# entn-at/tf-kaldi-speaker

Measured on AMD Instinct MI355X. Metric: utterances/sec x-vector extraction (30-dim x 300-frame), higher is better.
Workload: dtype f16+fp6-cross(f32-split); 1 GPU; tdnn x-vector (tdnn6_dense), statistics_pooling, 256 utt/GPU/step of 300 frames x 30 dims; batch_per_gpu=256, frames=300, node=tdnn6_dense, precision=f16f6, parallelism=utterance-shard x1, launch=stream launches

## Files before the change

### tf-kaldi-speaker_amd/csrc/pool.hip

```cpp
#include "xv_epilogue.h"

namespace xv {


__device__ __forceinline__ float act_apply(float v, int act, float alpha) {
  switch (act) {
    case ACT_RELU: return fmaxf(v, 0.0f);
    case ACT_LRELU: return fmaxf(v, kLreluAlpha * v);
    case ACT_PRELU: return fmaxf(v, 0.0f) + alpha * (v - fabsf(v)) * 0.5f;
    case ACT_TANH: return tanhf(v);
    default: return v;
  }
}

__device__ __forceinline__ float wave_sum(float v) {
#pragma unroll
  for (int o = 32; o > 0; o >>= 1) v += __shfl_xor(v, o, 64);
  return v;
}
__device__ __forceinline__ float wave_max(float v) {
#pragma unroll
  for (int o = 32; o > 0; o >>= 1) v = fmaxf(v, __shfl_xor(v, o, 64));
  return v;
}
// ... 40 lines not shown
  return hipGetLastError();
}

__global__ __launch_bounds__(256) void pool_finalize_kernel(const float* __restrict__ part, int C,
                                                            const int32_t* __restrict__ off0, int ctx,
                                                            const int32_t* __restrict__ slotbase,
                                                            float* __restrict__ out, int64_t ldo) {
  const int b = blockIdx.y;
  const int n = blockIdx.x * 256 + threadIdx.x;
  if (n >= C) return;
  const int r0 = off0[b] - b * ctx, r1 = off0[b + 1] - (b + 1) * ctx;
  const int t0 = r0 >> 6, t1 = (r1 - 1) >> 6;
  const int64_t base = (int64_t)slotbase[b];
  float s = 0.f;
  for (int t = t0; t <= t1; ++t) s += part[((base + t) * 2) * C + n];
  const float mean = s / (float)(r1 - r0);
  float m2 = 0.f;
  for (int t = t0; t <= t1; ++t) {
    const int ni = min(r1, (t + 1) << 6) - max(r0, t << 6);
    const float d = part[((base + t) * 2) * C + n] / (float)ni - mean;
    m2 += part[((base + t) * 2 + 1) * C + n] + (float)ni * d * d;
  }
  float var = m2 / (float)(r1 - r0);
  var = var <= kVarFloor ? kVarFloor : var;
  out[(int64_t)b * ldo + n] = mean;
  out[(int64_t)b * ldo + C + n] = sqrtf(var);
}

hipError_t launch_pool_finalize(const float* part, int C, const int32_t* off0, int B, int ctx,
                                const int32_t* slotbase, float* out, int64_t ldo, hipStream_t s) {
  if (B <= 0) return hipSuccess;
  hipLaunchKernelGGL(pool_finalize_kernel, dim3((C + 255) / 256, B), dim3(256), 0, s, part, C, off0, ctx, slotbase,
                     out, ldo);
  return hipGetLastError();
}

template <bool VEC>
__global__ __launch_bounds__(256) void stat_pool_kernel(const float* __restrict__ x, int64_t ldx, int C,
                                                        const int32_t* __restrict__ off0, int ctx,
                                                        float* __restrict__ out, int64_t ldo) {
  __shared__ float red[4][64];
  const int b = blockIdx.y;
  const int tid = threadIdx.x, lane = tid & 63, wave = tid >> 6;
  const int cl = tid & 15, rs = tid >> 4;
  const int col = blockIdx.x * 64 + cl * 4;
  const int r0 = off0[b] - b * ctx, r1 = off0[b + 1] - (b + 1) * ctx;
  const int L = r1 - r0;
  const float invL = 1.0f / (float)L;

  auto load4 = [&](int r) -> f32x4 {
    const float* p = x + (int64_t)r * ldx + col;
    if (VEC) {
      if (col < C) return *reinterpret_cast<const f32x4*>(p);
      return f32x4{0.f, 0.f, 0.f, 0.f};
    }
    f32x4 v;
#pragma unroll
    for (int e = 0; e < 4; ++e) v[e] = (col + e < C) ? p[e] : 0.f;
    return v;
  };
  auto block_sum = [&](f32x4 v) -> f32x4 {
#pragma unroll
    for (int e = 0; e < 4; ++e) {
      v[e] += __shfl_xor(v[e], 16, 64);
      v[e] += __shfl_xor(v[e], 32, 64);
    }
// ... 410 lines not shown
```

### tf-kaldi-speaker_amd/csrc/xv_kernels.h

```cpp
#pragma once
#include <hip/hip_runtime.h>
#include <stdint.h>

#include <string>

#include "../../include/xvec_hip.h"

namespace xv {

enum Act : int { ACT_NONE = 0, ACT_RELU = 1, ACT_LRELU = 2, ACT_PRELU = 3, ACT_TANH = 4 };

constexpr float kLreluAlpha = 0.2f;
constexpr int kFlagWords = 8, kUttSmallWord = 4, kFeatMaxSlots = 32768;
constexpr float kVarFloor = 1e-12f;

struct GemmArgs {
  const float* X;
  int64_t ldx;
  int cin;
  int M;
  int K;
  int N;
  const float* Wt;
  int Kpad;
// ... 40 lines not shown
  int64_t att_ld = 0;
  int att_heads = 0;
  const float* pool_w = nullptr;
  int pool_heads = 0;
  int pool_split = 0;
  int pool_dvh = 0;
  int pool_odim = 0;
};

hipError_t launch_gemm_f32(const GemmArgs& a, bool aligned, hipStream_t s);

int gemm_f32_ksplit(int M, int Kpad, int Npad);

int64_t gemm_bf16x3_tail_plan(int M, int Kpad, int Npad, int w, int* tail_mt, int* splits, int cb_quant = 1);

hipError_t launch_im2col_sb(const float* x, int64_t ldx, int cin, int w, int64_t rows, void* out_sb, int ldsb, int f16,
                            int* ovf, hipStream_t s);

hipError_t launch_gemm_bf16x3(const GemmArgs& a, hipStream_t s);
hipError_t launch_gemm_f16f6(const GemmArgs& a, hipStream_t s);
hipError_t launch_f6v2_tail_reduce(const GemmArgs& a, int nMain, hipStream_t s);
hipError_t launch_f6_from_sb(const void* sb, void* out, int64_t rows, int nblk, hipStream_t s);

hipError_t launch_build_rowmap(const int32_t* off0, int B, int ctx_in, int w, int32_t* rowmap, int M,
                               hipStream_t s);

hipError_t launch_stat_pool(const float* x, int64_t ldx, int C, const int32_t* off0, int B, int ctx,
                            float* out, int64_t ldo, hipStream_t s);

hipError_t launch_build_row2utt(const int32_t* off0, int B, int ctx, int32_t* row2utt, int M, hipStream_t s);
hipError_t launch_pool_finalize(const float* part, int C, const int32_t* off0, int B, int ctx,
                                const int32_t* slotbase, float* out, int64_t ldo, hipStream_t s);

hipError_t launch_build_rowmap_grid(const int32_t* off0, int B, int rows_per_t, int Fout, int So, int cover, int32_t* rowmap,
                                    int64_t M, hipStream_t s);
hipError_t launch_build_rowmap_grid_ts(const int32_t* off_in, const int32_t* off_out, int B, int rows_per_t, int Fout, int So,
                                       int ktime, int32_t* rowmap, int64_t M, hipStream_t s);
hipError_t launch_build_rowmap_grid_compact(const int32_t* off_in, const int32_t* off_out, int B, int Sin, int So, int Fout,
                                            int sw, int st, int ktime, int32_t* arow, int32_t* rowmap, int64_t M, int64_t Mpad,
                                            hipStream_t s);
hipError_t launch_grid_zero_border(const int32_t* off0, int B, int64_t frames, int F, int S, int chunks_y, int chunks_sb,
                                   float* y, void* ysb, hipStream_t s);
hipError_t launch_build_rowmap_rows(const int32_t* off0, int B, int32_t* rowmap, int64_t M, hipStream_t s);
hipError_t launch_build_rowmap_trows(const int32_t* off0, int B, int So, int32_t* rowmap, int64_t M, hipStream_t s);
hipError_t launch_build_rowmap_interior(const int32_t* off0, int B, int F, int S, int32_t* rowmap, int64_t M, hipStream_t s);
hipError_t launch_im2col2d_sb(const float* x, int64_t ldx, const int32_t* off0, int B, int F, int S, int64_t P, void* out_sb,
                              int f16, int* ovf, hipStream_t s);
hipError_t launch_im2col2d_f32(const float* x, int64_t ldx, const int32_t* off0, int B, int F, int S, int64_t P, float* out,
                               hipStream_t s);
hipError_t launch_conv0_direct(const float* x, int64_t ldx, const int32_t* off0, int B, int F, int S, int C, int64_t P,
                               const float* wdir, int act, const float* alpha, float* y, void* ysb, int ldsb, int f16, int* ovf,
                               float sb_mul, hipStream_t s);
hipError_t launch_grid_maxpool3x3(const float* x, const int32_t* off0, int B, int F, int S, int C, int64_t P, float* y,
                                  void* ysb, int ldsb, int f16, int* ovf, float sb_mul, hipStream_t s);
hipError_t launch_grid_unpad_n(const float* grid, const int32_t* off0, int B, int F, int S, int C, int64_t frames, float* out,
                               hipStream_t s);

hipError_t launch_cmn_select(const float* x, int64_t ld, int dim, const int32_t* off, int B, double* prefix,
                             const int32_t* src, int64_t out_rows, int window, int center, int min_window, float* out,
                             hipStream_t s);

int mfcc_create(const xv_mfcc_opts* opts, int device, xv_mfcc** out, std::string* err);
void mfcc_destroy(xv_mfcc* m);
int mfcc_num_frames(const xv_mfcc* m, int64_t num_samples, int64_t* out);
int mfcc_device(const xv_mfcc* m);
int mfcc_num_ceps(const xv_mfcc* m);
// ... 81 lines not shown
```

### tf-kaldi-speaker_amd/csrc/xvec_api.hip

```cpp
#include <hip/hip_runtime.h>

#include <algorithm>
#include <cmath>
#include <cstdarg>
#include <cstdio>
#include <cstring>
#include <map>
#include <mutex>
#include <string>
#include <vector>

#include "../../include/xvec_hip.h"
#include "xv_kernels.h"

using namespace xv;

namespace {

constexpr double kBnEps = 1e-3;
constexpr int kSlackRows = 512;
constexpr int kAlign = 256;

thread_local std::string g_last_error;

// ... 88 lines not shown

struct Op {
  int kind = OP_GEMM;
  int layer = -1;
  int in0 = -1, in1 = -1;
  int out = -1;
  int bnvec = -1;
};

struct Node {
  std::string name;
  int op = -1;
  int stage = -1;
  bool att_weights = false;
};

}

struct xv_handle {
  xv_model_desc desc{};
  int device = 0;
  bool finalized = false;
  std::string err;
  std::mutex mu;
  std::mutex err_mu;
  std::mutex prof_mu;
  int opt_pool_fusion = 1;
  int opt_tail_split = 1;
  int opt_onetap_f6_notail = 1;
  int opt_grid_f6 = 1;
  int opt_slab3 = 1;
  int opt_grid_compact = 1;
  int opt_att_fusion = 1;
  int opt_profile_dominant = 0;
  std::mutex pool_mu;
  std::vector<DevBuf> pool;
  size_t pool_bytes = 0;
  std::map<std::string, HostTensor> tensors;
  std::vector<Layer> layers;
  std::vector<Value> values;
  std::vector<Op> ops;
  std::vector<Node> nodes;
  DevBuf query;
  DevBuf ovf_flag;
  DevBuf query_eff;
  int key_npad = 0;
  int att_dk_h = 0, att_dk = 0, att_dv = 0;
  int final_ctx = 14;
  std::string post_bn_scope, post_alpha_name;
  DevBuf post_vec;
  int pool_dim = 0;
  struct ProfRec { hipEvent_t e0, e1; const xv_plan* plan; int step; };
  bool profiling = false;
  std::vector<hipEvent_t> prof_pool;
  size_t prof_next = 0;
  std::vector<ProfRec> prof_recs;
  int prof_forwards = 0;
};

struct PlanStep {
  int op = -1;
  int stage = -1;
  bool to_out = false;
  int64_t out_off = -1;
  int64_t out_sb_off = -1;
  int64_t in0_off = -1, in1_off = -1;
  int64_t in0_sb_off = -1;
  int64_t rows_in = 0, rows_out = 0;
  int M = 0;
  int rowmap = -1;
  int64_t scratch_off = -1;
  int64_t scratch2_off = -1;
  int ksplit = 1;
  int tail_mt = 0;
  bool fuse_pool = false;
  int lvl_in = 0, lvl_out = 0;
  int64_t frames_out = 0;
  bool grid_cover = false;
  bool out_f6 = false;
  bool trows = false;
  bool in_f6 = false;
  bool compact = false;
  int arow = -1;
  int fuse_att = 0;
  int64_t att_w_off = -1;
  int64_t att_s0_off = -1;
  int64_t att_ld = 0;
  bool unpad_to_out = false;
  int64_t flops = 0, bytes = 0;
};

struct xv_plan {
  xv_handle* h = nullptr;
  xv_plan_info info{};
  std::vector<int32_t> offsets;
  std::vector<int32_t> offsets_slotbase;
  DevBuf d_offsets;
  std::vector<int32_t> lvl_offsets[4];
  DevBuf d_lvl[4];
  const int32_t* dev_offsets(int level) const {
    return static_cast<const int32_t*>(level > 0 ? d_lvl[level].p : d_offsets.p);
  }
  DevBuf d_rowmaps;
  std::vector<int64_t> rowmap_off;
  std::vector<PlanStep> steps;
  DevBuf d_row2utt;
  DevBuf d_slotbase;
  int64_t pool_slots = 0;
  bool uniform_len = true;
  int uniform_L = 0;
  int dominant_step = 0;
};

namespace {

int fail(xv_handle* h, int code, const char* fmt, ...) {
  char buf[512];
  va_list ap;
  va_start(ap, fmt);
  vsnprintf(buf, sizeof(buf), fmt, ap);
  va_end(ap);
  if (h) {
    std::lock_guard<std::mutex> lk(h->err_mu);
    h->err = buf;
  }
  g_last_error = buf;
  return code;
}

#define XV_HIP(h, expr)                                                                              \
  do {                                                                                               \
    hipError_t _e = (expr);                                                                          \
    if (_e != hipSuccess)                                                                            \
      return fail((h), XV_ERR_HIP, "%s failed: %s (%s:%d)", #expr, hipGetErrorString(_e), __FILE__,  \
                  __LINE__);                                                                         \
  } while (0)

int64_t align_up(int64_t v, int64_t a) { return (v + a - 1) / a * a; }

constexpr size_t kPoolMaxBuffers = 96, kPoolMaxBytes = (size_t)1 << 30;
// ... 735 lines not shown
    }
    if (h->desc.att_apply_nonlinear) {
      const int n = h->pool_dim;
      std::vector<double> s, t;
      bn_fold(h, h->post_bn_scope, n, s, t);
      std::vector<float> vec((size_t)3 * n, 0.f);
      for (int i = 0; i < n; ++i) { vec[i] = (float)s[i]; vec[(size_t)n + i] = (float)t[i]; }
      if (!h->post_alpha_name.empty()) {
        const auto& a = T(h, h->post_alpha_name).data;
        for (int i = 0; i < n; ++i) vec[(size_t)2 * n + i] = a[i];
      }
      XV_HIP(h, h->post_vec.alloc(vec.size() * sizeof(float)));
      XV_HIP(h, hipMemcpy(h->post_vec.p, vec.data(), vec.size() * sizeof(float), hipMemcpyHostToDevice));
    }
  }
  XV_HIP(h, h->ovf_flag.alloc((kFlagWords + kFeatMaxSlots) * sizeof(int)));
  XV_HIP(h, hipMemset(h->ovf_flag.p, 0, (kFlagWords + kFeatMaxSlots) * sizeof(int)));
  XV_HIP(h, hipDeviceSynchronize());
  for (auto& kv : h->tensors) { kv.second.data.clear(); kv.second.data.shrink_to_fit(); }
  h->finalized = true;
  return XV_OK;
}

int xv_set_option(xv_handle* h, const char* name, int value) {
  if (!h || !name) return fail(h, XV_ERR_INVALID, "xv_set_option: null argument");
  std::lock_guard<std::mutex> lk(h->mu);
  if (!strcmp(name, "pool_fusion")) h->opt_pool_fusion = value != 0;
  else if (!strcmp(name, "tail_split")) h->opt_tail_split = value != 0;
  else if (!strcmp(name, "att_fusion")) h->opt_att_fusion = value != 0;
  else if (!strcmp(name, "slab3")) h->opt_slab3 = value != 0;
  else if (!strcmp(name, "onetap_f6_notail")) h->opt_onetap_f6_notail = value != 0;
  else if (!strcmp(name, "grid_f6")) h->opt_grid_f6 = value != 0;
  else if (!strcmp(name, "grid_compact")) h->opt_grid_compact = value != 0;
  else if (!strcmp(name, "profile_dominant")) h->opt_profile_dominant = value != 0;
  else return fail(h, XV_ERR_INVALID, "xv_set_option: unknown option '%s'", name);
  return XV_OK;
}

int xv_check_overflow(xv_handle* h, int reset) {
  if (!h) return fail(nullptr, XV_ERR_INVALID, "xv_check_overflow: null handle");
  if (!h->finalized || !h->ovf_flag.p) return 0;
  DeviceGuard g(h->device);
  std::vector<int32_t> w((size_t)kFlagWords + kFeatMaxSlots);
  XV_HIP(h, hipMemcpy(w.data(), h->ovf_flag.p, w.size() * sizeof(int32_t), hipMemcpyDeviceToHost));
  int32_t v[2] = {w[0], w[1]};
  for (int i = 0; i < kFeatMaxSlots; ++i) v[1] = std::max(v[1], w[(size_t)kFlagWords + i]);
  if (w[kUttSmallWord]) v[1] = w[kUttSmallWord];
  if (reset) XV_HIP(h, hipMemset(h->ovf_flag.p, 0, w.size() * sizeof(int32_t)));
  return xv_flags_decode(v);
}

int xv_flags_decode(const int32_t* flags) {
  if (!flags) return XV_ERR_INVALID;
  if (flags[0]) return 1;
  if (flags[1] > 0) {
    float mx;
    memcpy(&mx, &flags[1], 4);
    if (mx < 0.00390625f) return 2;
  }
  return 0;
}

int xv_flags_async(xv_handle* h, int32_t* host_flags, void* stream) {
  if (!h || !host_flags) return fail(h, XV_ERR_INVALID, "xv_flags_async: null argument");
  if (!h->finalized || !h->ovf_flag.p) { host_flags[0] = host_flags[1] = 0; return XV_OK; }
  DeviceGuard g(h->device);
// ... 150 lines not shown
  auto arena_free = [&](int64_t off, int64_t size) {
    free_list.push_back({off, size});
    std::sort(free_list.begin(), free_list.end(), [](const Block& a, const Block& b) { return a.off < b.off; });
    for (size_t i = 0; i + 1 < free_list.size();)
      if (free_list[i].off + free_list[i].size == free_list[i + 1].off) {
        free_list[i].size += free_list[i + 1].size;
        free_list.erase(free_list.begin() + i + 1);
      } else {
        ++i;
      }
  };

  std::vector<char> want_f32(h->values.size(), 0), want_sb(h->values.size(), 0);
  for (int o : order) {
    const Op& op = h->ops[o];
    const bool split_in = op.kind == OP_GEMM && h->layers[op.layer].use_split;
    if (op.in0 > 0) (split_in ? want_sb : want_f32)[op.in0] = 1;
    if (op.in1 > 0) want_f32[op.in1] = 1;
  }
  std::vector<int64_t> voff_sb(h->values.size(), -1), vsize_sb(h->values.size(), 0);

  int fused_value = -1;
  for (int o : order) {
    const Op& op = h->ops[o];
    if (op.kind != OP_STAT_POOL || op.in0 <= 0 || producer[op.in0] < 0) continue;
    const Op& prod = h->ops[producer[op.in0]];
    if (prod.kind != OP_GEMM || producer[op.in0] == node.op) continue;
    const Layer& L = h->layers[prod.layer];
    int readers = 0;
    for (int o2 : order)
      if (h->ops[o2].in0 == op.in0 || h->ops[o2].in1 == op.in0) ++readers;
    if (readers == 1 && L.w == 1 && (L.cout & 3) == 0 && h->opt_pool_fusion) fused_value = op.in0;
  }
  const int slot_value = fused_value >= 0 ? fused_value : att_pool_value;
  if (slot_value >= 0) {
    const int ctx = h->values[slot_value].ctx;
    const std::vector<int32_t>& so = lvl[h->values[slot_value].tlevel];
    std::vector<int32_t> slotbase(batch);
    int64_t nslots = 0;
    for (int b = 0; b < batch; ++b) {
      const int r0 = so[b] - b * ctx, r1 = so[b + 1] - (b + 1) * ctx;
      const int t0 = r0 >> 6, t1 = (r1 - 1) >> 6;
      slotbase[b] = (int32_t)(nslots - t0);
      nslots += t1 - t0 + 1;
    }
    p->pool_slots = nslots;
    p->offsets_slotbase = std::move(slotbase);
  }

  int64_t total_flops = 0;
  int64_t rowmap_elems = 0;
  for (size_t s = 0; s < order.size(); ++s) {
    const Op& op = h->ops[order[s]];
    PlanStep st;
    int64_t step_scratch = 0, step_scratch2 = 0;
    st.op = order[s];
    st.to_out = (order[s] == node.op);
    st.rows_in = op.in0 >= 0 ? value_rows(h, op.in0, Fl, batch) : 0;
    st.rows_out = value_rows(h, op.out, Fl, batch);
    st.lvl_in = op.in0 >= 0 ? h->values[op.in0].tlevel : 0;
    st.lvl_out = h->values[op.out].tlevel;
    st.frames_out = Fl[st.lvl_out];
    st.in0_off = op.in0 == 0 ? -2 : (op.in0 > 0 ? voff[op.in0] : -1);
    st.in0_sb_off = op.in0 > 0 ? voff_sb[op.in0] : -1;
    st.in1_off = op.in1 > 0 ? voff[op.in1] : -1;
    if (op.kind == OP_GEMM) {
      const Layer& L = h->layers[op.layer];
      st.stage = st.to_out ? node.stage : L.final_stage();
      const int64_t padded_rows = Fl[st.lvl_in] + 2 * (int64_t)batch;
      if (L.mode == 0) st.M = (int)(st.rows_in - (L.w - 1));
      else if (L.mode == 1 && L.use_f6) {
        st.trows = true;
        st.M = (int)padded_rows;
      }
      else if ((L.mode == 1 || L.mode == 2) && L.use_split && h->opt_grid_compact &&
               st.rows_in * (int64_t)sb_ld(L.cin) * 4 < ((int64_t)1 << 32)) {
        st.compact = true;
        st.M = (int)(Fl[st.lvl_out] * L.Fout);
      }
      else if (L.mode == 1 || L.mode == 2) st.M = (int)(padded_rows * (h->values[op.in0].grid_S / L.sw));
      else if (L.mode == 3) st.M = (int)padded_rows;
      else st.M = (int)(padded_rows * h->values[op.out].grid_S);
      if (st.compact || st.trows) st.grid_cover = false;
      else if (L.mode == 1 || L.mode == 2) st.grid_cover = L.st == 1 && h->values[op.in0].grid_S / L.sw == h->values[op.out].grid_S;
      else if (L.mode == 4) st.grid_cover = true;
      if (L.w > 1 || L.mode != 0) {
        st.rowmap = (int)p->rowmap_off.size();
        p->rowmap_off.push_back(rowmap_elems);
        rowmap_elems += align_up(st.M, 64);
        if (st.compact) {
          st.arow = (int)p->rowmap_off.size();
          p->rowmap_off.push_back(rowmap_elems);
          rowmap_elems += align_up(st.M, 128);
        }
      }
      const int64_t valid_out = L.mode == 0 ? st.rows_out : Fl[st.lvl_out] * (L.mode == 3 ? 1 : L.Fout);
      st.flops = 2 * valid_out * (int64_t)L.cout * L.K();
      st.bytes = 4 * (st.rows_in * L.cin + st.rows_out * L.cout + (int64_t)L.K() * L.cout);
      int64_t scratch = 0;
      if (L.mode == 4) {
        scratch = ((int64_t)st.M + kSlackRows) * 32 * 4;
      } else if (L.im2col) {
        scratch = L.cin_pad ? (st.rows_in + kSlackRows) * (int64_t)L.cin_pad * 4 : (st.M + kSlackRows) * (int64_t)L.Kpad * 4;
      } else if (!L.use_split && op.out != fused_value) {
        st.ksplit = gemm_f32_ksplit(st.M, L.Kpad, L.Npad);
        if (st.ksplit > 1) scratch = (int64_t)st.ksplit * st.M * L.Npad * 4;
      } else if (L.use_f6) {
        scratch = (st.rows_in + kSlackRows) * (int64_t)sb_ld(L.cin) * 4;
        if (h->opt_tail_split && op.in1 <= 0 && L.mode == 0) {
          const int64_t part = gemm_bf16x3_tail_plan(st.M, L.Kpad, L.Npad, L.w, &st.tail_mt, &st.ksplit, 4);
          if (part > 0) {
            step_scratch2 = align_up(part, kAlign);
            st.scratch2_off = arena_alloc(step_scratch2);
          }
        }
      } else if (L.use_split && L.mode == 0 && op.out != fused_value && op.in1 <= 0 && h->opt_tail_split &&
                 order[s] != key_prod && order[s] != val_prod) {
        scratch = gemm_bf16x3_tail_plan(st.M, L.Kpad, L.Npad, L.w, &st.tail_mt, &st.ksplit);
      }
      if (scratch > 0) {
        step_scratch = align_up(scratch, kAlign);
        st.scratch_off = arena_alloc(step_scratch);
      }
    } else if (op.kind == OP_AFFINE_ACT) {
      st.stage = st.to_out ? node.stage : 2;
      st.bytes = 8 * st.rows_out * h->values[op.out].cols;
    } else if (op.kind == OP_ATT_POOL && val_prod >= 0) {
      st.fuse_att = 1;
      st.bytes = 4 * (p->pool_slots * (2 * (h->pool_dim / 2) + h->desc.att_num_heads) + st.rows_out * h->values[op.out].cols);
      st.flops = 8 * p->pool_slots * (h->pool_dim / 2);
    } else if (op.kind == OP_STAT_POOL || op.kind == OP_ATT_POOL) {
      st.bytes = 4 * (st.rows_in * h->values[op.in0].cols + st.rows_out * h->values[op.out].cols);
      st.flops = 4 * st.rows_in * h->values[op.in0].cols;
      if (op.kind == OP_STAT_POOL && op.in0 == fused_value) {
        st.fuse_pool = true;
        st.bytes = 4 * (p->pool_slots * 2 * h->values[op.in0].cols + st.rows_out * h->values[op.out].cols);
// ... 40 lines not shown
        st.fuse_att = 2;
        vsize[op.out] = align_up(p->pool_slots * 2 * (int64_t)(h->pool_dim / 2) * 4, kAlign);
        voff[op.out] = arena_alloc(vsize[op.out]);
        st.out_off = voff[op.out];
        st.bytes = 4 * (st.rows_in * h->layers[op.layer].cin + (int64_t)h->layers[op.layer].K() * h->layers[op.layer].cout +
                        st.rows_out * h->desc.att_num_heads) + vsize[op.out];
        for (const PlanStep& prev : p->steps)
          if (h->ops[prev.op].kind == OP_ATT_SOFTMAX) { st.att_w_off = prev.out_off; st.att_s0_off = prev.att_s0_off; }
      } else if (op.out == fused_value) {
        st.fuse_pool = true;
        vsize[op.out] = align_up(p->pool_slots * 2 * (int64_t)h->values[op.out].cols * 4, kAlign);
        voff[op.out] = arena_alloc(vsize[op.out]);
        st.out_off = voff[op.out];
      } else if (want_f32[op.out] || node.att_weights) {
        vsize[op.out] = value_bytes(h, op.out, Fl, batch);
        if (op.kind == OP_ATT_SCORES && val_prod >= 0)
          vsize[op.out] = align_up(st.rows_out * (int64_t)h->desc.att_num_heads * 4, kAlign) +
                          align_up(p->pool_slots * (int64_t)h->desc.att_num_heads * 4, kAlign) + kAlign;
        voff[op.out] = arena_alloc(vsize[op.out]);
        st.out_off = voff[op.out];
      }
      if (want_sb[op.out]) {
        vsize_sb[op.out] = value_sb_bytes(h, op.out, Fl, batch);
        voff_sb[op.out] = arena_alloc(vsize_sb[op.out]);
        st.out_sb_off = voff_sb[op.out];
      }
    }
    if (op.kind == OP_ATT_POOL && val_prod >= 0)
      for (const PlanStep& prev : p->steps)
        if (h->ops[prev.op].kind == OP_ATT_SOFTMAX) st.att_s0_off = prev.att_s0_off;
    p->steps.push_back(st);
    if (step_scratch > 0) arena_free(st.scratch_off, step_scratch);
    if (step_scratch2 > 0) arena_free(st.scratch2_off, step_scratch2);
    for (int in : {op.in0, op.in1})
      if (in > 0 && last_use[in] == (int)s) {
        if (vsize[in] > 0) { arena_free(voff[in], vsize[in]); vsize[in] = 0; }
        if (vsize_sb[in] > 0) { arena_free(voff_sb[in], vsize_sb[in]); vsize_sb[in] = 0; }
      }
  }

  for (size_t i = 0; i < p->steps.size(); ++i)
    if (p->steps[i].flops > p->steps[p->dominant_step].flops) p->dominant_step = (int)i;

  for (PlanStep& cs : p->steps) {
    const Op& cop = h->ops[cs.op];
    if (cop.kind != OP_GEMM || !h->layers[cop.layer].use_f6) continue;
    const bool grid = h->layers[cop.layer].mode == 1;
    if (cs.in_f6) continue;
    int readers = 0;
    bool all_f6 = true;
    PlanStep* prod = nullptr;
    for (PlanStep& os : p->steps) {
      const Op& o = h->ops[os.op];
      if (o.in0 == cop.in0 || (!grid && o.in1 == cop.in0)) {
        ++readers;
        if (o.kind != OP_GEMM || !h->layers[o.layer].use_f6 || o.in0 != cop.in0) all_f6 = false;
      }
      if (o.out == cop.in0) prod = &os;
    }
    if (!prod || !all_f6 || (grid && readers != 1)) continue;
    const Op& pop = h->ops[prod->op];
    if (pop.kind != OP_GEMM) continue;
    const Layer& PL = h->layers[pop.layer];
    if (prod->to_out || prod->out_sb_off < 0 || prod->stage != PL.final_stage()) continue;
    if (grid) {
      const bool gather = PL.mode == 1 && !PL.use_f6 && PL.use_split && prod->compact && prod->out_off < 0 && pop.in1 <= 0;
// ... 62 lines not shown
      const Layer& L = h->layers[op.layer];
      const int ctx_in = h->values[op.in0].ctx;
      const int32_t* doff = p->dev_offsets(st.lvl_in);
      int32_t* rm = static_cast<int32_t*>(p->d_rowmaps.p) + p->rowmap_off[st.rowmap];
      if (L.mode == 0) e = launch_build_rowmap(doff, batch, ctx_in, L.w, rm, st.M, s);
      else if (st.trows) e = launch_build_rowmap_trows(doff, batch, h->values[op.out].grid_S, rm, st.M, s);
      else if (st.compact)
        e = launch_build_rowmap_grid_compact(doff, p->dev_offsets(st.lvl_out), batch, h->values[op.in0].grid_S,
                                             h->values[op.out].grid_S, L.Fout, L.sw, L.st, L.mode == 1 ? 3 : 1,
                                             static_cast<int32_t*>(p->d_rowmaps.p) + p->rowmap_off[st.arow], rm, st.M,
                                             align_up(st.M, 128), s);
      else if ((L.mode == 1 || L.mode == 2) && L.st == 2)
        e = launch_build_rowmap_grid_ts(doff, p->dev_offsets(st.lvl_out), batch, h->values[op.in0].grid_S / L.sw, L.Fout,
                                        h->values[op.out].grid_S, L.mode == 1 ? 3 : 1, rm, st.M, s);
      else if (L.mode == 1 || L.mode == 2)
        e = launch_build_rowmap_grid(doff, batch, h->values[op.in0].grid_S / L.sw, L.Fout, h->values[op.out].grid_S,
                                     st.grid_cover ? 1 : 0, rm, st.M, s);
      else if (L.mode == 3) e = launch_build_rowmap_rows(doff, batch, rm, st.M, s);
      else e = launch_build_rowmap_interior(doff, batch, L.Fout, h->values[op.out].grid_S, rm, st.M, s);
      if (e != hipSuccess) return bail(e, "build_rowmap");
    }
  }
  if (slot_value >= 0) {
    const int ctx = h->values[slot_value].ctx;
    const int64_t rows = value_rows(h, slot_value, Fl, batch);
    if ((e = pool_take(h, (size_t)rows * 4, p->d_row2utt)) != hipSuccess) return bail(e, "hipMalloc(row2utt)");
    if ((e = pool_take(h, (size_t)batch * 4, p->d_slotbase)) != hipSuccess) return bail(e, "hipMalloc(slotbase)");
    if ((e = hipMemcpyAsync(p->d_slotbase.p, p->offsets_slotbase.data(), (size_t)batch * 4, hipMemcpyHostToDevice, s)) != hipSuccess)
      return bail(e, "hipMemcpyAsync(slotbase)");
    if ((e = launch_build_row2utt(p->dev_offsets(h->values[slot_value].tlevel), batch, ctx,
                                  static_cast<int32_t*>(p->d_row2utt.p), (int)rows, s)) != hipSuccess)
      return bail(e, "build_row2utt");
  }
  *out = p;
  return XV_OK;
}

int xv_plan_query(const xv_plan* p, xv_plan_info* info) {
  if (!p || !info) return XV_ERR_INVALID;
  *info = p->info;
  return XV_OK;
}

void xv_plan_destroy(xv_plan* p) {
  if (!p) return;
  {
    DeviceGuard g(p->h->device);
    pool_give(p->h, p->d_offsets);
    for (int k = 1; k < 4; ++k) pool_give(p->h, p->d_lvl[k]);
    pool_give(p->h, p->d_rowmaps);
    pool_give(p->h, p->d_row2utt);
    pool_give(p->h, p->d_slotbase);
  }
  delete p;
}

static const char* step_name(const xv_handle* h, const PlanStep& st) {
  const Op& op = h->ops[st.op];
  switch (op.kind) {
    case OP_GEMM: {
      const Layer& L = h->layers[op.layer];
      if (!L.ep[ST_AFFINE].empty()) return L.ep[ST_AFFINE].c_str();
      const size_t a = L.kernel_name.find('/'), b = L.kernel_name.rfind('/');
      static thread_local std::string tmp;
      tmp = (a != std::string::npos && b > a) ? L.kernel_name.substr(a + 1, b - a - 1) : L.kernel_name;
      return tmp.c_str();
    }
    case OP_STAT_POOL: return "stat_pool";
    case OP_ATT_SCORES: return "att_scores";
    case OP_ATT_SOFTMAX: return "att_softmax";
    case OP_ATT_POOL: return "att_pool";
    case OP_AFFINE_ACT: return "att_post";
    case OP_L2_SCALE: return "l2_scale";
    case OP_GRID_MAXPOOL: return "conv0_max";
    default: return "op";
  }
}

static int run_plan(xv_handle* h, const xv_plan* p, const float* feats, int feat_ld, float* out, int64_t out_cap,
                    void* workspace, int64_t ws_bytes, hipStream_t s) {
  if (!h || !p) return fail(h, XV_ERR_INVALID, "xv_forward: null handle/plan");
  if (p->h != h) return fail(h, XV_ERR_INVALID, "xv_forward: plan belongs to another handle");
  if (!feats || !out) return fail(h, XV_ERR_INVALID, "xv_forward: null feature/output pointer");
  if (feat_ld < h->desc.feat_dim) return fail(h, XV_ERR_INVALID, "xv_forward: feat_ld %d < feature_dim %d", feat_ld, h->desc.feat_dim);
  if (out_cap < p->info.out_rows * p->info.out_cols)
// ... 84 lines not shown
          a.ntaps = L.mode == 1 ? 3 : 1;
          a.ktap = L.mode == 1 ? 3 * L.cin : (L.mode == 2 ? L.cin : L.Fin * L.cin);
          a.tap_stride = Sin * L.cin;
          a.cin = a.K;
        }
        if (op.in1 > 0) { a.R = in_ptr(st.in1_off); a.ldr = L.cout; }
        if (st.fuse_att == 1) {
          a.Y = nullptr;
          a.att_part = reinterpret_cast<float*>(ws + st.out_off);
          a.att_ld = st.att_ld;
          a.att_heads = d.att_num_heads;
          a.att_q = static_cast<const float*>(h->query_eff.p);
        } else if (st.fuse_att == 2) {
          a.Y = nullptr;
          a.pool_part = reinterpret_cast<float*>(ws + st.out_off);
          a.pool_row2utt = static_cast<const int32_t*>(p->d_row2utt.p);
          a.pool_slotbase = static_cast<const int32_t*>(p->d_slotbase.p);
          a.pool_w = reinterpret_cast<const float*>(ws + st.att_w_off);
          a.pool_heads = d.att_num_heads;
          a.pool_split = d.att_split_value;
          a.pool_dvh = d.att_split_value ? L.cout / d.att_num_heads : L.cout;
          a.pool_odim = h->pool_dim / 2;
        }
        if (st.fuse_pool) {
          a.Y = nullptr;
          a.pool_part = reinterpret_cast<float*>(ws + st.out_off);
          a.pool_row2utt = static_cast<const int32_t*>(p->d_row2utt.p);
          a.pool_slotbase = static_cast<const int32_t*>(p->d_slotbase.p);
        }
        if (st.out_sb_off >= 0) {
          a.Ysb = ws + st.out_sb_off;
          a.ldsb = sb_ld(L.cout);
          if (st.out_off < 0 && !st.to_out) a.Y = nullptr;
        }
        if (L.mode == 4) {
          if (st.scratch_off < 0) return fail(h, XV_ERR_STATE, "conv0 has no scratch");
          a.cin = 32; a.K = 32;
          const bool direct = L.use_split && !st.to_out && st.stage == L.final_stage() && L.cout % 8 == 0 &&
                              (st.out_sb_off < 0 || L.cout % 32 == 0) && L.cout <= 256 && L.wdir.p;
          if (direct) {
            XV_HIP(h, launch_conv0_direct(feats, feat_ld, off, B, L.Fout, vo.grid_S, L.cout, st.M, static_cast<const float*>(L.wdir.p),
                                          L.act, L.d_alpha(), st.out_off >= 0 ? reinterpret_cast<float*>(ws + st.out_off) : nullptr,
                                          st.out_sb_off >= 0 ? ws + st.out_sb_off : nullptr, sb_ld(L.cout), f16,
                                          static_cast<int*>(h->ovf_flag.p), a.sb_mul, s));
            break;
          }
          if (L.use_split) {
            XV_HIP(h, launch_im2col2d_sb(feats, feat_ld, off, B, L.Fout, vo.grid_S, st.M, ws + st.scratch_off, f16, static_cast<int*>(h->ovf_flag.p), s));
            a.Xsb = ws + st.scratch_off; a.ldsbx = 32; a.Wsb = L.wsb.p; a.Wfr = L.wfr.p;
            XV_HIP(h, launch_gemm_bf16x3(a, s));
          } else {
            XV_HIP(h, launch_im2col2d_f32(feats, feat_ld, off, B, L.Fout, vo.grid_S, st.M, reinterpret_cast<float*>(ws + st.scratch_off), s));
            a.X = reinterpret_cast<const float*>(ws + st.scratch_off); a.ldx = 32;
            XV_HIP(h, launch_gemm_f32(a, true, s));
          }
          if (st.unpad_to_out)
            XV_HIP(h, launch_grid_unpad_n(reinterpret_cast<const float*>(ws + st.out_off), off_out, B, vo.grid_F, vo.grid_S, vo.cols,
                                          st.frames_out, out, s));
          break;
        }
        if (L.im2col) {
          if (st.scratch_off < 0) return fail(h, XV_ERR_STATE, "im2col layer has no scratch");
          if (L.cin_pad) {
            XV_HIP(h, launch_im2col_sb(feats, feat_ld, L.cin, 1, st.rows_in, ws + st.scratch_off, L.cin_pad, f16,
                                       static_cast<int*>(h->ovf_flag.p), s));
            if (f16) XV_HIP(h, launch_feat_utt_guard(feats, feat_ld, L.cin, off, B, static_cast<int*>(h->ovf_flag.p), s));
// ... 600 lines not shown
```

Baseline: 216,300 utterances/s.

## Fuse pooling finalize into following dense GEMM with split-K last-block reduction

Adds a head_fused kernel that computes per-utterance mean/std from pooled partial sums directly into LDS and immediately multiplies them by the next dense layer's weights using fp32 MFMA. The channel dimension is split across blocks, and a per-utterance-tile atomic counter lets the last block sum the slab partials and apply the affine epilogue and activation. This removes the separate pool_finalize launch, the write and re-read of the pooled stats, and the standalone GEMM launch. In exchange it adds scratch slabs, atomic counters that must be reset, and cross-block synchronisation.

Result: slower. 214,000 utterances/s (-1.0%).

```diff
diff --git a/tf-kaldi-speaker_amd/csrc/pool.hip b/tf-kaldi-speaker_amd/csrc/pool.hip
--- a/tf-kaldi-speaker_amd/csrc/pool.hip
+++ b/tf-kaldi-speaker_amd/csrc/pool.hip
@@ -96,6 +96,201 @@
   if (B <= 0) return hipSuccess;
   hipLaunchKernelGGL(pool_finalize_kernel, dim3((C + 255) / 256, B), dim3(256), 0, s, part, C, off0, ctx, slotbase,
                      out, ldo);
+  return hipGetLastError();
+}
+
+constexpr int kHeadU = 16, kHeadMaxCS = 256, kHeadBatch = 8;
+
+void head_fused_shape(int B, int C, int* nU, int* nS, int* CS) {
+  const int nu = (B + kHeadU - 1) / kHeadU;
+  int target = 256 / nu;
+  target = target < 1 ? 1 : (target > 32 ? 32 : target);
+  int cs = ((C + target - 1) / target + 15) / 16 * 16;
+  cs = cs < 16 ? 16 : (cs > kHeadMaxCS ? kHeadMaxCS : cs);
+  *nU = nu;
+  *CS = cs;
+  *nS = (C + cs - 1) / cs;
+}
+
+int64_t head_fused_scratch_bytes(int B, int C, int Npad) {
+  int nU, nS, CS;
+  head_fused_shape(B, C, &nU, &nS, &CS);
+  return (int64_t)nU * nS * kHeadU * Npad * 4;
+}
+
+int head_fused_counters(int B) { return (B + kHeadU - 1) / kHeadU; }
+
+struct HeadPair {
+  const float* col;
+  int r0, r1;
+  int64_t base;
+};
+
+__device__ __forceinline__ void head_finish(const HeadPair& q, int C, const float (&sv)[kHeadBatch], const float (&mv)[kHeadBatch],
+                                            float& mean_out, float& std_out) {
+  const int r0 = q.r0, r1 = q.r1;
+  const int t0 = r0 >> 6, t1 = (r1 - 1) >> 6, n = t1 - t0 + 1;
+  const float L = (float)(r1 - r0);
+  auto term = [&](int t, float s1, float m2, float mean) {
+    const int ni = min(r1, (t + 1) << 6) - max(r0, t << 6);
+    const float d = s1 / (float)ni - mean;
+    return m2 + (float)ni * d * d;
+  };
+  float s = 0.f, m2 = 0.f;
+#pragma unroll
+  for (int i = 0; i < kHeadBatch; ++i) s += i < n ? sv[i] : 0.f;
+  for (int t = t0 + kHeadBatch; t <= t1; ++t) s += q.col[((q.base + t) * 2) * C];
+  const float mean = s / L;
+#pragma unroll
+  for (int i = 0; i < kHeadBatch; ++i) m2 += i < n ? term(t0 + i, sv[i], mv[i], mean) : 0.f;
+  for (int t = t0 + kHeadBatch; t <= t1; ++t) m2 += term(t, q.col[((q.base + t) * 2) * C], q.col[((q.base + t) * 2 + 1) * C], mean);
+  float var = m2 / L;
+  var = var <= kVarFloor ? kVarFloor : var;
+  mean_out = mean;
+  std_out = sqrtf(var);
+}
+
+__global__ __launch_bounds__(256) void head_fused_kernel(GemmArgs p, const float* __restrict__ part, int C,
+                                                         const int32_t* __restrict__ off0, int ctx,
+                                                         const int32_t* __restrict__ slotbase, int* __restrict__ counters,
+                                                         int nU, int nS, int CS) {
+  __shared__ __attribute__((aligned(16))) float As[kHeadU * (2 * kHeadMaxCS + 4) + 4];
+  const int tid = threadIdx.x, lane = tid & 63, wave = tid >> 6;
+  const int xcd = blockIdx.x & 7, rest = blockIdx.x >> 3;
+  const int ut = rest % nU, sl = (rest / nU) * 8 + xcd;
+  if (sl >= nS) return;
+  const int B = p.M;
+  const int c0 = sl * CS, cs = min(CS, C - c0);
+  const int ldA = 2 * CS + 4;
+
+  constexpr int P = 4;
+  const int total = kHeadU * CS;
+  for (int idx0 = tid; idx0 < total; idx0 += 256 * P) {
+    HeadPair q[P];
+    bool ok[P];
+    float sv[P][kHeadBatch], mv[P][kHeadBatch];
+#pragma unroll
+    for (int j = 0; j < P; ++j) {
+      const int idx = idx0 + 256 * j;
+      const int u = idx / CS, c = idx - u * CS;
+      const int b = ut * kHeadU + u;
+      ok[j] = idx < total && b < B && c < cs;
+      const int bb = ok[j] ? b : ut * kHeadU, cc = ok[j] ? c : 0;
+      q[j].r0 = off0[bb] - bb * ctx;
+      q[j].r1 = off0[bb + 1] - (bb + 1) * ctx;
+      q[j].base = (int64_t)slotbase[bb];
+      q[j].col = part + c0 + cc;
+    }
+#pragma unroll
+    for (int j = 0; j < P; ++j) {
+      const int t0 = q[j].r0 >> 6, t1 = (q[j].r1 - 1) >> 6;
+#pragma unroll
+      for (int i = 0; i < kHeadBatch; ++i) {
+        const int64_t t = q[j].base + min(t0 + i, t1);
+        sv[j][i] = q[j].col[(t * 2) * C];
+        mv[j][i] = q[j].col[(t * 2 + 1) * C];
+      }
+    }
+#pragma unroll
+    for (int j = 0; j < P; ++j) {
+      const int idx = idx0 + 256 * j;
+      if (idx >= total) break;
+      float mean, sd;
+      head_finish(q[j], C, sv[j], mv[j], mean, sd);
+      const int u = idx / CS, c = idx - u * CS;
+      As[u * ldA + c] = ok[j] ? mean : 0.f;
+      As[u * ldA + CS + c] = ok[j] ? sd : 0.f;
+    }
+  }
+  __syncthreads();
+
+  const int r16 = lane & 15, g = lane >> 4;
+  const int nb = (cs + 15) >> 4, nhb = 2 * nb;
+  float* slab = p.partial + ((int64_t)(ut * nS + sl) * kHeadU) * p.Npad;
+  for (int n0 = wave * 128; n0 < p.Npad; n0 += 512) {
+    f32x4 acc[8];
+#pragma unroll
+    for (int t = 0; t < 8; ++t) acc[t] = f32x4{0.f, 0.f, 0.f, 0.f};
+    const float* wrow = p.Wt + (int64_t)(n0 + r16) * p.Kpad;
+    f32x4 wc[8], wn[8], ac, an;
+    auto load_block = [&](int hb, f32x4 (&w)[8], f32x4& a) {
+      const int half = hb >= nb ? 1 : 0;
+      const int cl = (hb - half * nb) * 16 + 4 * g;
+      const int k = min((half ? C : 0) + c0 + cl, p.Kpad - 4);
+#pragma unroll
+      for (int t = 0; t < 8; ++t) w[t] = *reinterpret_cast<const f32x4*>(wrow + (int64_t)t * 16 * p.Kpad + k);
+      a = *reinterpret_cast<const f32x4*>(As + r16 * ldA + half * CS + cl);
+    };
+    load_block(0, wc, ac);
+    for (int hb = 0; hb < nhb; ++hb) {
+      if (hb + 1 < nhb) load_block(hb + 1, wn, an);
+#pragma unroll
+      for (int j = 0; j < 4; ++j)
+#pragma unroll
+        for (int t = 0; t < 8; ++t) acc[t] = __builtin_amdgcn_mfma_f32_16x16x4f32(wc[t][j], ac[j], acc[t], 0, 0, 0);
+#pragma unroll
+      for (int t = 0; t < 8; ++t) wc[t] = wn[t];
+      ac = an;
+    }
+#pragma unroll
+    for (int t = 0; t < 8; ++t) *reinterpret_cast<f32x4*>(slab + (int64_t)r16 * p.Npad + n0 + t * 16 + 4 * g) = acc[t];
+  }
+
+  asm volatile("s_waitcnt vmcnt(0)" ::: "memory");
+  __syncthreads();
+  float* flag = As + kHeadU * (2 * kHeadMaxCS + 4);
+  if (tid == 0) {
+    __builtin_amdgcn_fence(__ATOMIC_RELEASE, "agent");
+    asm volatile("s_waitcnt vmcnt(0)" ::: "memory");
+    const int ticket = __hip_atomic_fetch_add(counters + ut, 1, __ATOMIC_RELAXED, __HIP_MEMORY_SCOPE_AGENT);
+    const bool last = ticket == nS - 1;
+    if (last) {
+      __builtin_amdgcn_fence(__ATOMIC_ACQUIRE, "agent");
+      asm volatile("s_waitcnt vmcnt(0)" ::: "memory");
+      __hip_atomic_store(counters + ut, 0, __ATOMIC_RELAXED, __HIP_MEMORY_SCOPE_AGENT);
+    }
+    *flag = last ? 1.f : 0.f;
+  }
+  __syncthreads();
+  if (*flag == 0.f) return;
+
+  const int rows = min(kHeadU, B - ut * kHeadU);
+  const int n4 = (p.N + 3) >> 2;
+  const float* tile = p.partial + ((int64_t)ut * nS * kHeadU) * p.Npad;
+  const int64_t slab_stride = (int64_t)kHeadU * p.Npad;
+  for (int idx = tid; idx < rows * n4; idx += 256) {
+    const int u = idx / n4, n = (idx - u * n4) * 4;
+    const float* src = tile + (int64_t)u * p.Npad + n;
+    f32x4 acc = {0.f, 0.f, 0.f, 0.f};
+    int s = 0;
+    for (; s + 8 <= nS; s += 8) {
+      f32x4 v[8];
+#pragma unroll
+      for (int i = 0; i < 8; ++i) v[i] = *reinterpret_cast<const f32x4*>(src + (s + i) * slab_stride);
+#pragma unroll
+      for (int i = 0; i < 8; ++i) acc += v[i];
+    }
+    for (; s < nS; ++s) acc += *reinterpret_cast<const f32x4*>(src + s * slab_stride);
+    const int m = ut * kHeadU + u;
+    bool zero;
+    const int orow = out_row(p, m, zero);
+    if (orow < 0) continue;
+#pragma unroll
+    for (int e = 0; e < 4; ++e) {
+      if (n + e >= p.N) break;
+      const float v = fmaf(acc[e], p.scale[n + e], p.shift[n + e]);
+      p.Y[(int64_t)orow * p.ldy + n + e] = zero ? 0.f : apply_act(v, p.act, p.alpha ? p.alpha[n + e] : 0.f);
+    }
+  }
+}
+
+hipError_t launch_head_fused(const GemmArgs& a, const float* part, int C, const int32_t* off0, int ctx,
+                             const int32_t* slotbase, int* counters, hipStream_t s) {
+  if (a.M <= 0) return hipSuccess;
+  int nU, nS, CS;
+  head_fused_shape(a.M, C, &nU, &nS, &CS);
+  const int grid = ((nS + 7) / 8) * 8 * nU;
+  hipLaunchKernelGGL(head_fused_kernel, dim3(grid), dim3(256), 0, s, a, part, C, off0, ctx, slotbase, counters, nU, nS, CS);
   return hipGetLastError();
 }
 
diff --git a/tf-kaldi-speaker_amd/csrc/xv_kernels.h b/tf-kaldi-speaker_amd/csrc/xv_kernels.h
--- a/tf-kaldi-speaker_amd/csrc/xv_kernels.h
+++ b/tf-kaldi-speaker_amd/csrc/xv_kernels.h
@@ -96,6 +96,11 @@
 hipError_t launch_pool_finalize(const float* part, int C, const int32_t* off0, int B, int ctx,
                                 const int32_t* slotbase, float* out, int64_t ldo, hipStream_t s);
 
+int64_t head_fused_scratch_bytes(int B, int C, int Npad);
+int head_fused_counters(int B);
+hipError_t launch_head_fused(const GemmArgs& a, const float* part, int C, const int32_t* off0, int ctx,
+                             const int32_t* slotbase, int* counters, hipStream_t s);
+
 hipError_t launch_build_rowmap_grid(const int32_t* off0, int B, int rows_per_t, int Fout, int So, int cover, int32_t* rowmap,
                                     int64_t M, hipStream_t s);
 hipError_t launch_build_rowmap_grid_ts(const int32_t* off_in, const int32_t* off_out, int B, int rows_per_t, int Fout, int So,
diff --git a/tf-kaldi-speaker_amd/csrc/xvec_api.hip b/tf-kaldi-speaker_amd/csrc/xvec_api.hip
--- a/tf-kaldi-speaker_amd/csrc/xvec_api.hip
+++ b/tf-kaldi-speaker_amd/csrc/xvec_api.hip
@@ -144,6 +144,7 @@
   int opt_slab3 = 1;
   int opt_grid_compact = 1;
   int opt_att_fusion = 1;
+  int opt_head_fusion = 1;
   int opt_profile_dominant = 0;
   std::mutex pool_mu;
   std::vector<DevBuf> pool;
@@ -198,6 +199,10 @@
   int64_t att_w_off = -1;
   int64_t att_s0_off = -1;
   int64_t att_ld = 0;
+  bool head_fused = false;
+  int head_lvl = 0;
+  int head_ctx = 0;
+  int head_cols = 0;
   bool unpad_to_out = false;
   int64_t flops = 0, bytes = 0;
 };
@@ -218,6 +223,7 @@
   std::vector<PlanStep> steps;
   DevBuf d_row2utt;
   DevBuf d_slotbase;
+  DevBuf d_headcnt;
   int64_t pool_slots = 0;
   bool uniform_len = true;
   int uniform_L = 0;
@@ -1019,6 +1025,7 @@
   else if (!strcmp(name, "onetap_f6_notail")) h->opt_onetap_f6_notail = value != 0;
   else if (!strcmp(name, "grid_f6")) h->opt_grid_f6 = value != 0;
   else if (!strcmp(name, "grid_compact")) h->opt_grid_compact = value != 0;
+  else if (!strcmp(name, "head_fusion")) h->opt_head_fusion = value != 0;
   else if (!strcmp(name, "profile_dominant")) h->opt_profile_dominant = value != 0;
   else return fail(h, XV_ERR_INVALID, "xv_set_option: unknown option '%s'", name);
   return XV_OK;
@@ -1235,6 +1242,25 @@
       if (h->ops[o2].in0 == op.in0 || h->ops[o2].in1 == op.in0) ++readers;
     if (readers == 1 && L.w == 1 && (L.cout & 3) == 0 && h->opt_pool_fusion) fused_value = op.in0;
   }
+  int head_pool_op = -1, head_gemm_op = -1;
+  if (h->opt_head_fusion && fused_value >= 0 && batch <= 512) {
+    for (int o : order) {
+      const Op& op = h->ops[o];
+      if (op.kind != OP_STAT_POOL || op.in0 != fused_value || o == node.op) continue;
+      int reader = -1;
+      if (readers_of(op.out) != 1) continue;
+      for (int o2 : order)
+        if (h->ops[o2].in0 == op.out || h->ops[o2].in1 == op.out) reader = o2;
+      const Op& rd = h->ops[reader];
+      if (rd.kind != OP_GEMM || rd.in0 != op.out || rd.in1 > 0 || want_sb[rd.out]) continue;
+      const Layer& L = h->layers[rd.layer];
+      const int C = h->values[fused_value].cols;
+      if (L.use_split || L.use_f6 || L.im2col || L.mode != 0 || L.w != 1 || L.K() != 2 * C || (C & 3) || h->values[rd.out].grid_F > 0)
+        continue;
+      head_pool_op = o;
+      head_gemm_op = reader;
+    }
+  }
   const int slot_value = fused_value >= 0 ? fused_value : att_pool_value;
   if (slot_value >= 0) {
     const int ctx = h->values[slot_value].ctx;
@@ -1255,6 +1281,10 @@
   int64_t rowmap_elems = 0;
   for (size_t s = 0; s < order.size(); ++s) {
     const Op& op = h->ops[order[s]];
+    if (order[s] == head_pool_op) {
+      total_flops += 6 * p->pool_slots * h->values[fused_value].cols;
+      continue;
+    }
     PlanStep st;
     int64_t step_scratch = 0, step_scratch2 = 0;
     st.op = order[s];
@@ -1305,6 +1335,15 @@
         scratch = ((int64_t)st.M + kSlackRows) * 32 * 4;
       } else if (L.im2col) {
         scratch = L.cin_pad ? (st.rows_in + kSlackRows) * (int64_t)L.cin_pad * 4 : (st.M + kSlackRows) * (int64_t)L.Kpad * 4;
+      } else if (order[s] == head_gemm_op) {
+        const Value& fv = h->values[fused_value];
+        st.head_fused = true;
+        st.head_lvl = fv.tlevel;
+        st.head_ctx = fv.ctx;
+        st.head_cols = fv.cols;
+        st.in0_off = voff[fused_value];
+        scratch = head_fused_scratch_bytes(st.M, fv.cols, L.Npad);
+        st.bytes += 4 * (p->pool_slots * 2 * fv.cols + st.rows_in * 2 * (int64_t)fv.cols);
       } else if (!L.use_split && op.out != fused_value) {
         st.ksplit = gemm_f32_ksplit(st.M, L.Kpad, L.Npad);
         if (st.ksplit > 1) scratch = (int64_t)st.ksplit * st.M * L.Npad * 4;
@@ -1411,6 +1450,7 @@
     p->steps.push_back(st);
     if (step_scratch > 0) arena_free(st.scratch_off, step_scratch);
     if (step_scratch2 > 0) arena_free(st.scratch2_off, step_scratch2);
+    if (st.head_fused && vsize[fused_value] > 0) { arena_free(voff[fused_value], vsize[fused_value]); vsize[fused_value] = 0; }
     for (int in : {op.in0, op.in1})
       if (in > 0 && last_use[in] == (int)s) {
         if (vsize[in] > 0) { arena_free(voff[in], vsize[in]); vsize[in] = 0; }
@@ -1539,6 +1579,11 @@
                                   static_cast<int32_t*>(p->d_row2utt.p), (int)rows, s)) != hipSuccess)
       return bail(e, "build_row2utt");
   }
+  if (head_gemm_op >= 0) {
+    const size_t bytes = (size_t)head_fused_counters(batch) * 4;
+    if ((e = pool_take(h, bytes, p->d_headcnt)) != hipSuccess) return bail(e, "hipMalloc(head counters)");
+    if ((e = hipMemsetAsync(p->d_headcnt.p, 0, bytes, s)) != hipSuccess) return bail(e, "hipMemsetAsync(head counters)");
+  }
   *out = p;
   return XV_OK;
 }
@@ -1558,6 +1603,7 @@
     pool_give(p->h, p->d_rowmaps);
     pool_give(p->h, p->d_row2utt);
     pool_give(p->h, p->d_slotbase);
+    pool_give(p->h, p->d_headcnt);
   }
   delete p;
 }
@@ -1708,6 +1754,13 @@
           a.Ysb = ws + st.out_sb_off;
           a.ldsb = sb_ld(L.cout);
           if (st.out_off < 0 && !st.to_out) a.Y = nullptr;
+        }
+        if (st.head_fused) {
+          if (st.scratch_off < 0 || !p->d_headcnt.p) return fail(h, XV_ERR_STATE, "fused segment head has no scratch / counters");
+          a.partial = reinterpret_cast<float*>(ws + st.scratch_off);
+          XV_HIP(h, launch_head_fused(a, in_ptr(st.in0_off), st.head_cols, p->dev_offsets(st.head_lvl), st.head_ctx,
+                                      static_cast<const int32_t*>(p->d_slotbase.p), static_cast<int*>(p->d_headcnt.p), s));
+          break;
         }
         if (L.mode == 4) {
           if (st.scratch_off < 0) return fail(h, XV_ERR_STATE, "conv0 has no scratch");
```
